# swami1995/diff-qp-mpc

Hardware: AMD Instinct MI355X
Metric: QPs/sec (fwd+bwd), batch=4096 n=3 m=3 T=5 (higher is better)
Workload: dtype f64; 1 GPU; random dense QP family R (SURVEY 8d), configs[0] shape at the BASELINE metric batch: B=4096/GPU nz=30 nineq=30 neq=15; global_batch=4096, n_state=3, n_ctrl=3, T=5, parallelism=batch-shard x1, termination=batch (the reference's batch-coupled rule, parity-safe)

## Files before the change

diff-qp-mpc_amd/_lib.py:

```python
import ctypes
import os

from . import _build

_dp = ctypes.c_void_p


class dqp_dims(ctypes.Structure):
    _fields_ = [("nbatch", ctypes.c_int32), ("nz", ctypes.c_int32), ("nineq", ctypes.c_int32),
                ("neq", ctypes.c_int32),
                ("stride_Q", ctypes.c_int64), ("stride_p", ctypes.c_int64),
                ("stride_G", ctypes.c_int64), ("stride_h", ctypes.c_int64),
                ("stride_A", ctypes.c_int64), ("stride_b", ctypes.c_int64)]


class dqp_opts(ctypes.Structure):
    _fields_ = [("eps", ctypes.c_double), ("stall_tol", ctypes.c_double),
                ("max_iter", ctypes.c_int32),
                ("not_improved_lim", ctypes.c_int32), ("flags", ctypes.c_uint32),
                ("reserved", ctypes.c_int32),
                ("dyn_id", ctypes.c_int32), ("dyn_T", ctypes.c_int32), ("dyn_dt", ctypes.c_double),
                ("dyn_x0", ctypes.c_void_p)]


DQP_OK = 0
DQP_FLAG_DENSE_BACKWARD = 1
DQP_FLAG_GENERIC_ONLY = 2
DQP_FLAG_NO_NULLSPACE = 4
DQP_FLAG_RIC_GLOBAL_WS = 64
DQP_FLAG_BACKWARD_CTX = 8
DQP_FLAG_BATCH_TERMINATION = 16
DQP_FLAG_HISTORY_ONLY = 32
DQP_FLAG_STRICT_GET_STEP = 128
DQP_FLAG_STAGEWISE = 256
DQP_STATUS_Q_NOT_PD = 1
DQP_STATUS_A_RANK_DEF = 2
DQP_MAX_DIM = 64
DQP_MAX_DIM_LARGE = 512
SHARED_GRAD_KC = 64

SYMBOLS = ("dqp_version", "dqp_error_string", "dqp_workspace_bytes", "dqp_termination_bytes",
           "dqp_qp_forward", "dqp_qp_backward", "dqp_qp_backward_shared_bytes", "dqp_qp_backward_shared", "dqp_term_local_masks", "dqp_qp_forward_finish", "dqp_mpc_assemble", "dqp_mpc_assemble_backward",
           "dqp_mpc_qp_supported", "dqp_mpc_qp_workspace_bytes", "dqp_mpc_qp_host_n_state", "dqp_mpc_qp_termination_bytes", "dqp_mpc_qp_forward", "dqp_mpc_qp_backward", "dqp_mpc_line_search", "dqp_mpc_rollout_backward",
           "dqp_al_newton_step", "dqp_al_chol_solve", "dqp_al_assemble", "dqp_al_merit",
           "dqp_al_newton_solve_bytes", "dqp_al_newton_solve",
           "dqp_al_outer_update", "dqp_al_banded_factor_bytes", "dqp_al_banded_newton_step", "dqp_al_banded_solve",
           "dqp_al_banded_newton_step_jac", "dqp_al_banded_jac_factor_bytes", "dqp_al_lane_group", "dqp_al_mpc_solve_bytes", "dqp_al_mpc_solve",
           "dqp_al_mpc_solve_fused_supported", "dqp_al_mpc_solve_fused_bytes", "dqp_al_mpc_solve_fused",
           "dqp_mpc_qp_stepped_workspace_bytes", "dqp_mpc_qp_stepped_termination_bytes", "dqp_mpc_qp_forward_stepped", "dqp_trace_begin", "dqp_trace_end",
           "dqp_dyn_sizes", "dqp_dyn_step", "dqp_dyn_jacobian", "dqp_dyn_forward_dynamics",
           "dqp_dyn_forward_derivatives")
DQP_DYN = {"pendulum1l": 1, "cartpole1l": 2, "cartpole2l": 3, "pendulum_euler": 4, "pendulum_dx": 5,
           "rexquadrotor": 6, "integrator": 7}


class dqp_al_mpc_dims(ctypes.Structure):
    _fields_ = [("nbatch", ctypes.c_int32), ("n_state", ctypes.c_int32), ("n_ctrl", ctypes.c_int32),
                ("T", ctypes.c_int32)]


class dqp_al_dims(ctypes.Structure):
    _fields_ = [("nbatch", ctypes.c_int32), ("nz", ctypes.c_int32), ("ncon", ctypes.c_int32),
                ("reserved", ctypes.c_int32)]


class dqp_mpc_dims(ctypes.Structure):
    _fields_ = [("nbatch", ctypes.c_int32), ("n_state", ctypes.c_int32), ("n_ctrl", ctypes.c_int32),
                ("T", ctypes.c_int32), ("has_bounds", ctypes.c_int32), ("dyn_id", ctypes.c_int32),
                ("n_state_host", ctypes.c_int32)]



class dqp_trace_record(ctypes.Structure):
    _fields_ = [("kernel", ctypes.c_char * 248), ("ms", ctypes.c_float), ("reserved", ctypes.c_int32)]


_lib = None


def path():
    return os.environ.get("DQP_HIP_LIBRARY") or _build.SO


def load():
    global _lib
    if _lib is not None:
        return _lib
    so = path()
    if not os.path.exists(so):
        raise RuntimeError(
            "diff_qp_mpc_amd: %s is missing. Build it with `python -c 'import __graft_entry__ as g; "
            "g.build()'` (hipcc --offload-arch=gfx950). There is no CPU fallback." % so)
    try:
        lib = ctypes.CDLL(so)
    except OSError as e:
        raise RuntimeError("diff_qp_mpc_amd: cannot load %s: %s" % (so, e))
    lib.dqp_version.restype = ctypes.c_int
    lib.dqp_error_string.restype = ctypes.c_char_p
    lib.dqp_error_string.argtypes = [ctypes.c_int]
    lib.dqp_workspace_bytes.restype = ctypes.c_size_t
    lib.dqp_workspace_bytes.argtypes = [ctypes.POINTER(dqp_dims)]
    lib.dqp_qp_forward.restype = ctypes.c_int
    lib.dqp_termination_bytes.restype = ctypes.c_size_t
    lib.dqp_termination_bytes.argtypes = [ctypes.POINTER(dqp_dims), ctypes.POINTER(dqp_opts)]
    lib.dqp_qp_forward.argtypes = [ctypes.POINTER(dqp_dims), ctypes.POINTER(dqp_opts)] + [_dp] * 15
    lib.dqp_term_local_masks.restype = ctypes.c_int
    lib.dqp_term_local_masks.argtypes = [ctypes.POINTER(dqp_dims), ctypes.POINTER(dqp_opts)] + [_dp] * 3
    lib.dqp_qp_forward_finish.restype = ctypes.c_int
    lib.dqp_qp_forward_finish.argtypes = [ctypes.POINTER(dqp_dims), ctypes.POINTER(dqp_opts)] + [_dp] * 16
    lib.dqp_qp_backward.restype = ctypes.c_int
    lib.dqp_qp_backward.argtypes = [ctypes.POINTER(dqp_dims), ctypes.POINTER(dqp_opts)] + [_dp] * 17
    lib.dqp_qp_backward_shared_bytes.restype = ctypes.c_size_t
    lib.dqp_qp_backward_shared_bytes.argtypes = [ctypes.POINTER(dqp_dims)]
    lib.dqp_qp_backward_shared.restype = ctypes.c_int
    lib.dqp_qp_backward_shared.argtypes = [ctypes.POINTER(dqp_dims), ctypes.POINTER(dqp_opts)] + [_dp] * 18
    lib.dqp_mpc_assemble.restype = ctypes.c_int
    lib.dqp_mpc_assemble.argtypes = [ctypes.POINTER(dqp_mpc_dims)] + [_dp] * 14
# ... 115 lines not shown
```

diff-qp-mpc_amd/csrc/dqp_common.h:

```cpp
#ifndef DQP_COMMON_H_
#define DQP_COMMON_H_
#include <hip/hip_runtime.h>
#include <stdint.h>

#include "../../include/dqp.h"
#include "dqp_trace.h"

namespace dqp {

constexpr int WAVE = 64;

struct KParams {
    const double *Q, *p, *G, *h, *A, *b;
    long long sQ, sp, sG, sh, sA, sb;
    double *zhat, *lam, *nu, *slack, *best_resid;
    const double *zin, *lamin, *nuin, *slackin, *gin;
    double *dQ, *dp, *dG, *dh, *dA, *db;
    int32_t *info;
    double *workspace;
    unsigned long long *stamps;
    int B, N, M, E;
    int ldz, ldm, lde, ldt;
    double eps, stallTol;
    int maxIter, notImprovedLim;
    unsigned flags;
    double *hist;
    const int32_t *cap;
    int histIters;
    int dynId, dynT, dynN, dynM;
    double dynDt;
    const double *dynX0;
    const double *mC, *mc, *mF, *mf, *mx0, *mul, *muu;
    double *mdC, *mdc, *mdF, *mdf, *mdx0;
    int mn, mm, mT;
    double *snap;
    const double *histIn;
    const double *extRy;
    int itBegin, itEnd;
};

constexpr int TERM_HDR = 8;

constexpr int TERM_MAXIT = 64;
constexpr int TERM_ACC_BYTES = 3 * 8 + TERM_HDR * 4;

__device__ __forceinline__ void hist_put(const KParams &P, long long qp, int it, double resid, double mu)
{
    double2 *h = reinterpret_cast<double2 *>(P.hist) + (long long)it * P.B + qp;
    *h = make_double2(resid, mu);
}
__device__ __forceinline__ void hist_fill(const KParams &P, long long qp, int iters)
{
    const double nan = __builtin_nan("");
    for (int it = iters; it < P.histIters; ++it)
        reinterpret_cast<double2 *>(P.hist)[(long long)it * P.B + qp] = make_double2(nan, nan);
}
__device__ __forceinline__ void term_zero_acc(const KParams &P)
{
    if (P.hist && blockIdx.x == 0) {
        unsigned *a = reinterpret_cast<unsigned *>(P.hist + (long long)P.B * P.histIters * 2);
        for (int i = threadIdx.x; i < TERM_ACC_BYTES / 4; i += blockDim.x) a[i] = 0u;
    }
}

__device__ __forceinline__ bool term_flagged(const KParams &P, long long qp) { return P.cap[TERM_HDR + qp] >= P.cap[0]; }

size_t term_bytes(int B, int maxIter, int snapDim);
int term_decide(const KParams &P, void *term, void *stream);
int term_local_masks(const KParams &P, void *term, unsigned long long *masks, void *stream);
int term_decide_global(const KParams &P, void *term, const unsigned long long *masks, void *stream);
void term_bind_pass1(KParams &P, void *term, int snapDim);
void term_bind_pass2(KParams &P, void *term);


#ifdef DQP_STAMPS
extern unsigned long long *g_debug_stamps;
#endif
int r16_forward(const KParams &P, void *stream);
int r16_backward(const KParams &P, void *stream);
int r16n_forward(const KParams &P, void *stream);
long long r16n_workspace_doubles(int N, int M, int E);
int r16n_snapshot_doubles(int N, int M, int E);
bool ric_supported(int n_state, int n_ctrl);
long long ric_workspace_doubles(int n_state, int n_ctrl, int T);
int ric_forward(const KParams &P, void *stream);
long long ric_stepped_workspace_doubles(int n_state, int n_ctrl, int T, int B);
int ric_forward_stepped(const KParams &P, void *stream);
int ric_backward(const KParams &P, void *stream);
int ric_snapshot_doubles(int n_state, int n_ctrl, int T);
int ric_finish(const KParams &P, void *stream);
bool ricw_supported(int n_state, int n_ctrl);
long long ricw_workspace_doubles(int n_state, int n_ctrl, int T);
int ricw_forward(const KParams &P, void *stream);
long long ricw_stepped_workspace_doubles(int n_state, int n_ctrl, int T, int B);
int ricw_forward_stepped(const KParams &P, void *stream);
int ricw_backward(const KParams &P, void *stream);
int ricw_snapshot_doubles(int n_state, int n_ctrl, int T);
#define DQP_RIC_HOST16_SIZES X(15, 1) X(14, 2) X(13, 3) X(11, 5) X(10, 6) X(9, 7) X(8, 8)
#define DQP_RIC_HOSTW_SIZES X(31, 1) X(30, 2) X(29, 3) X(28, 4) X(27, 5) X(26, 6) X(25, 7)
#define DQP_RIC_HOST_SIZES DQP_RIC_HOST16_SIZES DQP_RIC_HOSTW_SIZES
#define DQP_RIC_HOST_PART_IDS PART(0) PART(1) PART(2) PART(3) PART(4) PART(5) PART(6) PART(7) PART(8)
enum { RIC_HOST_FORWARD = 0, RIC_HOST_STEPPED = 1, RIC_HOST_BACKWARD = 2 };
#define PART(k) int ric_host_run_##k(int op, const KParams &P, void *stream);
DQP_RIC_HOST_PART_IDS
#undef PART
bool stage_supported(int n_state, int n_ctrl);
bool stage_native(int n_state, int n_ctrl);
int stage_q(int n_state, int n_ctrl);
long long stage_layout_doubles(int n_state, int n_ctrl, int T);
int stage_forward(const KParams &P, void *stream);
int stage_forward_stepped(const KParams &P, void *stream);
int stage_backward(const KParams &P, void *stream);
struct PadRegion {
    double *C, *F, *c, *tau, *g, *dc, *f, *df, *nu, *ry, *x0, *dx0, *dC, *dF;
};
long long pad_kernel_doubles(int n_host, int n_ctrl, int T, int B, bool stepped);
long long pad_region_doubles(int n_host, int n_ctrl, int T, int B);
PadRegion pad_region(double *base, int n_host, int n_ctrl, int T, int B);
int pad_pack(int n, int n_host, int m, int T, int B, const PadRegion &R, const double *C, const double *c, const double *F,
             const double *f, const double *x0, const double *tau, const double *nu, const double *g, const double *ry,
             void *stream);
int pad_unpack(int n, int n_host, int m, int T, int B, const PadRegion &R, double *tau, double *nu, double *dC, double *dc,
               double *dF, double *df, double *dx0, void *stream);
long long big_workspace_doubles(int N, int M, int E);
bool big_fits(int N, int M, int E);
int big_forward(const KParams &P, void *stream);
int big_backward(const KParams &P, void *stream);

int al_banded_newton_step_keep(const dqp_al_mpc_dims *d, int dyn_id, double dt, const double *xu, const double *x0,
                               const double *Qdiag, const double *q, const double *lam, const double *rho,
                               const double *u_lower, const double *u_upper, double *update, void *factor, int32_t *info,
                               void *stream, int keep);
int r16n_backward(const KParams &P, void *stream);

}
#endif
```

diff-qp-mpc_amd/csrc/dqp_pdipm.hip:

```cpp

#include <hip/hip_runtime.h>
#include <math.h>
#include <stdint.h>

#include "dqp_common.h"
#include "dqp_dyn_models.h"

using namespace dqp;

namespace {

#define WSYNC() __syncthreads()

__device__ __forceinline__ double bcast(double v, int src)
{
    int lo = __double2loint(v), hi = __double2hiint(v);
    lo = __builtin_amdgcn_readlane(lo, src);
    hi = __builtin_amdgcn_readlane(hi, src);
    return __hiloint2double(hi, lo);
}

template <int CTRL> __device__ __forceinline__ double dppd(double v)
{
    return __builtin_amdgcn_update_dpp(v, v, CTRL, 0xf, 0xf, true);
// ... 641 lines not shown
template <typename K>
int launch(K kernel, const KParams &P, size_t lds_bytes, void *stream)
{
    if (P.B == 0) return DQP_OK;
    if (lds_bytes > 64 * 1024) {
        if (hipFuncSetAttribute(reinterpret_cast<const void *>(kernel),
                                hipFuncAttributeMaxDynamicSharedMemorySize,
                                (int)lds_bytes) != hipSuccess)
            return DQP_ERR_LAUNCH;
    }
    DQP_LAUNCH(kernel, dim3(P.B), dim3(WAVE), lds_bytes, (hipStream_t)stream, P);
    return hipGetLastError() == hipSuccess ? DQP_OK : DQP_ERR_LAUNCH;
}

}

#ifdef DQP_STAMPS
namespace dqp { unsigned long long *g_debug_stamps = nullptr; }
#endif

extern "C" {

#ifdef DQP_STAMPS
__attribute__((visibility("default"))) void dqp_debug_set_stamps(void *dev_ptr)
{
    dqp::g_debug_stamps = (unsigned long long *)dev_ptr;
}
#endif

__attribute__((visibility("default"))) int dqp_version(void) { return DQP_VERSION; }

__attribute__((visibility("default"))) const char *dqp_error_string(int code)
{
    switch (code) {
    case DQP_OK: return "ok";
    case DQP_ERR_BAD_ARG: return "bad argument";
    case DQP_ERR_TOO_LARGE: return "problem too large for the fused one-wavefront kernels";
    case DQP_ERR_LAUNCH: return "HIP kernel launch failed";
    case DQP_ERR_NO_DEVICE: return "no HIP device";
    default: return "unknown error";
    }
}

__attribute__((visibility("default"))) size_t dqp_workspace_bytes(const dqp_dims *d)
{
    if (!d || d->nbatch <= 0) return 0;
    if (d->nz > DQP_MAX_DIM || d->nineq > DQP_MAX_DIM || d->neq > DQP_MAX_DIM) {
        if (d->nz > DQP_MAX_DIM_LARGE || d->nineq > DQP_MAX_DIM_LARGE || d->neq > DQP_MAX_DIM_LARGE) return 0;
        return (size_t)d->nbatch * (size_t)dqp::big_workspace_doubles(d->nz, d->nineq, d->neq) * sizeof(double);
    }
    return (size_t)d->nbatch * (size_t)dqp::r16n_workspace_doubles(d->nz, d->nineq, d->neq) * sizeof(double);
}

__attribute__((visibility("default"))) size_t
dqp_termination_bytes(const dqp_dims *d, const dqp_opts *o)
{
    if (!d || d->nbatch <= 0 || !o || !(o->flags & DQP_FLAG_BATCH_TERMINATION)) return 0;
    return dqp::term_bytes(d->nbatch, o->max_iter, dqp::r16n_snapshot_doubles(d->nz, d->nineq, d->neq));
}

static int forward_once(const KParams &P, size_t lds, void *workspace, void *stream);

__attribute__((visibility("default"))) int
dqp_qp_forward(const dqp_dims *dims, const dqp_opts *opts, const double *Q, const double *p,
               const double *G, const double *h, const double *A, const double *b, double *zhat,
               double *lam, double *nu, double *slack, int32_t *info, double *best_resid,
               void *workspace, void *termination, void *stream)
{
    KParams P = {};
    size_t lds = 0;
    int rc = fill_params(dims, opts, P, lds);
    if (rc != DQP_OK) return rc;
    if (P.B == 0) return DQP_OK;
    if (!Q || !p || !G || !h || !zhat || !lam || !slack) return DQP_ERR_BAD_ARG;
    P.workspace = (double *)workspace;
    if (P.E > 0 && (!A || !b || !nu)) return DQP_ERR_BAD_ARG;
    P.Q = Q; P.p = p; P.G = G; P.h = h; P.A = A; P.b = b;
    P.zhat = zhat; P.lam = lam; P.nu = nu; P.slack = slack;
    P.info = info; P.best_resid = best_resid;
    if (!(P.flags & DQP_FLAG_BATCH_TERMINATION)) return forward_once(P, lds, workspace, stream);
    if (!termination || P.maxIter < 1 || P.maxIter > 64) return DQP_ERR_BAD_ARG;
    P.eps = opts ? opts->eps : 1e-12;
    const bool nullspace = workspace && !(P.flags & (DQP_FLAG_GENERIC_ONLY | DQP_FLAG_NO_NULLSPACE)) && !P.dynId && !is_big(P);
    term_bind_pass1(P, termination, nullspace ? r16n_snapshot_doubles(P.N, P.M, P.E) : 0);
    if ((rc = forward_once(P, lds, workspace, stream)) != DQP_OK) return rc;
    if (P.flags & DQP_FLAG_HISTORY_ONLY) return DQP_OK;
    if ((rc = term_decide(P, termination, stream)) != DQP_OK) return rc;
    term_bind_pass2(P, termination);
    return forward_once(P, lds, workspace, stream);
}

__attribute__((visibility("default"))) int
dqp_term_local_masks(const dqp_dims *dims, const dqp_opts *opts, void *termination, uint64_t *masks, void *stream)
{
    KParams P = {};
    size_t lds = 0;
    int rc = fill_params(dims, opts, P, lds);
    if (rc != DQP_OK) return rc;
    if (!(P.flags & DQP_FLAG_BATCH_TERMINATION) || !termination || !masks || P.maxIter < 1 || P.maxIter > 64)
        return DQP_ERR_BAD_ARG;
    if (P.B == 0) return hipMemsetAsync(masks, 0, 24, (hipStream_t)stream) == hipSuccess ? DQP_OK : DQP_ERR_LAUNCH;
    P.eps = opts ? opts->eps : 1e-12;
    return term_local_masks(P, termination, (unsigned long long *)masks, stream);
}

__attribute__((visibility("default"))) int
dqp_qp_forward_finish(const dqp_dims *dims, const dqp_opts *opts, const double *Q, const double *p,
                      const double *G, const double *h, const double *A, const double *b, double *zhat,
                      double *lam, double *nu, double *slack, int32_t *info, double *best_resid,
                      void *workspace, void *termination, const uint64_t *masks, void *stream)
{
    KParams P = {};
    size_t lds = 0;
    int rc = fill_params(dims, opts, P, lds);
    if (rc != DQP_OK) return rc;
    if (P.B == 0) return DQP_OK;
    if (!(P.flags & DQP_FLAG_BATCH_TERMINATION) || !termination || !masks || P.maxIter < 1 || P.maxIter > 64)
        return DQP_ERR_BAD_ARG;
    if (!Q || !p || !G || !h || !zhat || !lam || !slack) return DQP_ERR_BAD_ARG;
    if (P.E > 0 && (!A || !b || !nu)) return DQP_ERR_BAD_ARG;
    P.workspace = (double *)workspace;
    P.Q = Q; P.p = p; P.G = G; P.h = h; P.A = A; P.b = b;
    P.zhat = zhat; P.lam = lam; P.nu = nu; P.slack = slack;
    P.info = info; P.best_resid = best_resid;
    P.eps = opts ? opts->eps : 1e-12;
    const bool nullspace = workspace && !(P.flags & (DQP_FLAG_GENERIC_ONLY | DQP_FLAG_NO_NULLSPACE)) && !P.dynId && !is_big(P);
    term_bind_pass1(P, termination, nullspace ? r16n_snapshot_doubles(P.N, P.M, P.E) : 0);
    if ((rc = term_decide_global(P, termination, (const unsigned long long *)masks, stream)) != DQP_OK) return rc;
    term_bind_pass2(P, termination);
    return forward_once(P, lds, workspace, stream);
}

static int forward_once(const KParams &P, size_t lds, void *workspace, void *stream)
{
    int rc;
    if (is_big(P)) return workspace ? big_forward(P, stream) : DQP_ERR_BAD_ARG;
    if (!(P.flags & DQP_FLAG_GENERIC_ONLY) && !P.dynId) {
        rc = (workspace && !(P.flags & DQP_FLAG_NO_NULLSPACE)) ? r16n_forward(P, stream) : 1;
        if (rc == 1) rc = r16_forward(P, stream);
        if (rc != 1) return rc;
    }
    const int mx = P.N > P.M ? (P.N > P.E ? P.N : P.E) : (P.M > P.E ? P.M : P.E);
    if (mx <= 16) return launch(qp_forward_kernel<16>, P, lds, stream);
    if (mx <= 32) return launch(qp_forward_kernel<32>, P, lds, stream);
    return launch(qp_forward_kernel<64>, P, lds, stream);
}

enum { MPC_NONE = 0, MPC_R16N = 1, MPC_RIC = 2, MPC_RICW = 3, MPC_PAD = 4 };

static long long stage_ws_doubles(int n, int m, int T)
{
    return ric_supported(n, m) ? ric_workspace_doubles(n, m, T) : ricw_workspace_doubles(n, m, T);
}

static int mpc_params(const dqp_mpc_dims *md, const dqp_opts *opts, KParams &P, size_t &lds, int &kind)
{
    kind = MPC_NONE;
    if (!md || md->T < 2 || md->n_state < 1 || md->n_ctrl < 1 || !md->has_bounds || md->nbatch < 0) return DQP_ERR_BAD_ARG;
    dqp_dims d = {};
    d.nbatch = md->nbatch;
    d.nz = md->T * (md->n_state + md->n_ctrl);
    d.nineq = 2 * md->T * md->n_ctrl;
    d.neq = md->T * md->n_state;
    if (md->n_state_host) {
        const int np = md->n_state_host, m = md->n_ctrl;
        if (md->dyn_id || np < md->n_state || !stage_supported(np, m)) return DQP_ERR_BAD_ARG;
        if (md->T > 200000 || stage_layout_doubles(np, m, md->T) * 8 * 4 > 0x7fffffffLL) return DQP_ERR_TOO_LARGE;
        P.stamps = nullptr;
        P.B = d.nbatch; P.N = md->T * (np + m); P.M = d.nineq; P.E = md->T * np;
        fill_opts(opts, P);
// ... 286 lines not shown
```

diff-qp-mpc_amd/csrc/dqp_r16n.hip:

```cpp

#include "dqp_r16_prims.h"

namespace dqp {
namespace r16n {

using namespace dqp::r16;

template <int N_, int M_, int E_> struct Cfg {
    static constexpr int N = N_, M = M_, E = E_, R = N_ - E_;
    static constexpr int SN = slots(N_), SM = slots(M_), SR = slots(N_ - E_);
    static constexpr int SE = E_ > 0 ? slots(E_) : 1, EC = E_ > 0 ? E_ : 1;
    static constexpr bool PARK = slots(N_) >= 3;
#ifndef DQP_R16N_PARK_WU
#define DQP_R16N_PARK_WU 1
#endif
    static constexpr bool PARKWU = PARK || DQP_R16N_PARK_WU;
#ifndef DQP_R16N_PIN_ALL
#define DQP_R16N_PIN_ALL 1
#endif
    static constexpr bool PIN = PARK || DQP_R16N_PIN_ALL;
#ifndef DQP_R16N_SPLIT_ALL
#define DQP_R16N_SPLIT_ALL 0
#endif
    static constexpr bool SPLIT = PARK || DQP_R16N_SPLIT_ALL;
// ... 829 lines not shown
        if (r == 0) {
            if (P.info) { P.info[2 * qp] = st.status; P.info[2 * qp + 1] = iters; }
            if (P.best_resid) P.best_resid[qp] = best;
        }
    }
}

template <class C>
__global__ __launch_bounds__(64) void forward_kernel(KParams P)
{
    constexpr int N = C::N, M = C::M, E = C::E, R = C::R;
    constexpr int SN = C::SN, SM = C::SM, SE = C::SE, SR = C::SR;
    extern __shared__ __attribute__((aligned(16))) double sm[];
    const int lane = threadIdx.x, r = lane & 15, qrow = lane >> 4;
    long long qp = (long long)blockIdx.x * 4 + qrow;
    bool live = qp < P.B;
    if (!live) qp = P.B - 1;
    int maxIter = P.maxIter;
    const bool batch = (P.flags & DQP_FLAG_BATCH_TERMINATION) != 0;
    const bool strict = (P.flags & DQP_FLAG_STRICT_GET_STEP) != 0;
    if (P.cap) {
        maxIter = min(maxIter, P.cap[0]);
        live = live && term_flagged(P, qp);
        if (__builtin_amdgcn_ballot_w64(live) == 0) return;
    }
    double *lds = sm + qrow * C::ldsQPpad;
    double *dummy = lds + C::oDummy + r;

    term_zero_acc(P);
    State<C> st;
    STAMP(P, 0);
    setup<C>(P, qp, r, lds, st);
    STAMP(P, 15);

    bool inM[SM], inR[SR];
#pragma unroll
    for (int s = 0; s < SM; ++s) inM[s] = r + 16 * s < M;
#pragma unroll
    for (int s = 0; s < SR; ++s) inR[s] = r + 16 * s < R;

    double T[SM][M], rdu[SM];
    double w[SR], s_[SM], z[SM];
    double cc = 1.0, delta = 0.0;
    {
        double one[SM], hp[SM], cp[SR], g[SM], gtz[SR];
#pragma unroll
        for (int s = 0; s < SM; ++s) one[s] = inM[s] ? 1.0 : 0.0;
        vec_get<SM>(lds + C::oHp, hp, M, r);
        vec_get<SR>(lds + C::oCp, cp, R, r);
        mul_Gz<C>(st, cp, g);
#pragma unroll
        for (int s = 0; s < SM; ++s) g[s] = inM[s] ? -hp[s] - g[s] : 0.0;
        __builtin_amdgcn_sched_barrier(0);
        factor_T<C>(lds, T, st.rdiag, one, rdu, r);
        lu_solve<SM, M>(T, rdu, g, r);
        __builtin_amdgcn_sched_barrier(0);
        mul_GzT<C>(st, g, gtz, r);
#pragma unroll
        for (int s = 0; s < SR; ++s) w[s] = inR[s] ? -cp[s] - gtz[s] : 0.0;
        double ms = INFINITY, mz = INFINITY;
#pragma unroll
        for (int s = 0; s < SM; ++s) {
            z[s] = inM[s] ? g[s] : 0.0;
            s_[s] = -z[s];
            ms = fmin(ms, inM[s] ? s_[s] : INFINITY);
            mz = fmin(mz, inM[s] ? z[s] : INFINITY);
        }
        ms = row_min(ms); mz = row_min(mz);
#pragma unroll
        for (int s = 0; s < SM; ++s) {
            if (ms < 0.0 && inM[s]) s_[s] -= ms - 1.0;
            if (mz < 0.0 && inM[s]) z[s] -= mz - 1.0;
        }
        delta = mz < 0.0 ? 1.0 - mz : 0.0;
        if (r == 0) P.workspace[qp * (long long)C::wsQP + C::wDl] = delta;
    }

    double gz[SR];
    mul_GzT<C>(st, z, gz, r);
    STAMP(P, 6);
    double best = INFINITY, bestc = 1.0;
    bool have_best = false, done = false;
    int nNot = 0, iters = 0;

    for (int it = 0; it < maxIter; ++it) {
        double rw[SR], rz[SM];
        {
            double cp[SR], hp[SM], gw[SM];
            vec_get<SR>(lds + C::oCp, cp, R, r);
            vec_get<SM>(lds + C::oHp, hp, M, r);
            mul_Gz<C>(st, w, gw);
#pragma unroll
            for (int s = 0; s < SR; ++s) rw[s] = inR[s] ? w[s] + cp[s] + gz[s] : 0.0;
#pragma unroll
            for (int s = 0; s < SM; ++s) rz[s] = inM[s] ? gw[s] + s_[s] - hp[s] : 0.0;
        }
        double sz = 0.0, nz2 = 0.0;
#pragma unroll
        for (int s = 0; s < SM; ++s) { sz = fma(s_[s], z[s], sz); nz2 = fma(rz[s], rz[s], nz2); }
        double nx2 = rx_norm2_partial<C>(st, lds, rw, cc * delta, r);
        sz = row_sum(sz); nz2 = row_sum(nz2); nx2 = row_sum(nx2);
        const double mu = fabs(sz * (1.0 / M));
        const double resid = sqrt(nz2) + sqrt(nx2) + M * mu;
        if (!done) {
            iters = it + 1;
            if (!have_best || resid < best) {
                nNot = 0; have_best = true; best = resid; bestc = cc;
                vec_put<SR>(lds + C::oBw, w, R, r, dummy);
                vec_put<SM>(lds + C::oBs, s_, M, r, dummy);
                vec_put<SM>(lds + C::oBz, z, M, r, dummy);
                if (P.snap && live) {
                    double *sp = P.snap + ((long long)it * P.B + qp) * C::snapDim;
#pragma unroll
                    for (int s = 0; s < SR; ++s)
                        if (inR[s]) sp[r + 16 * s] = w[s];
#pragma unroll
                    for (int s = 0; s < SM; ++s)
                        if (inM[s]) { sp[R + r + 16 * s] = s_[s]; sp[R + M + r + 16 * s] = z[s]; }
                    if (r == 0) sp[R + 2 * M] = cc;
                }
            } else {
                nNot += 1;
            }
            if (batch) {
                if (P.hist && r == 0 && live) hist_put(P, qp, it, resid, mu);
                done = !(fabs(resid) < INFINITY);
            } else if ((nNot >= P.notImprovedLim && best < P.stallTol) || best < P.eps || mu > 1e32 ||
                       !(fabs(resid) < INFINITY))
                done = true;
        }
        if (__builtin_amdgcn_ballot_w64(!done) == 0) break;
        if (it == 1) STAMP(P, 9);

        double dza[SM], dsa[SM];
        {
            double gu[SM];
            mul_Gz<C>(st, rw, gu);
#pragma unroll
            for (int s = 0; s < SM; ++s) dza[s] = rz[s] - s_[s] - gu[s];
        }
        __builtin_amdgcn_sched_barrier(0);
        double dinv[SM];
#pragma unroll
        for (int s = 0; s < SM; ++s) dinv[s] = inM[s] ? s_[s] * frcp(z[s]) : 0.0;
        factor_T<C>(lds, T, st.rdiag, dinv, rdu, r);
        if (it == 1) STAMP(P, 10);
        lu_solve<SM, M>(T, rdu, dza, r);
        if (it == 1) STAMP(P, 11);
        double rzv[SM], rsv[SM];
#pragma unroll
        for (int s = 0; s < SM; ++s) {
            rzv[s] = inM[s] ? frcp(z[s]) : 0.0;
            rsv[s] = inM[s] ? frcp(s_[s]) : 0.0;
        }
        double tm = 0.0;
#pragma unroll
        for (int s = 0; s < SM; ++s) {
            dsa[s] = (-z[s] - dza[s]) * dinv[s];
            tm = fmax(tm, fmax(-dza[s] * rzv[s], -dsa[s] * rsv[s]));
        }
        bool zero_step = false;
        if (strict) {
#pragma unroll
            for (int s = 0; s < SM; ++s) zero_step |= inM[s] && (dza[s] == 0.0 || dsa[s] == 0.0);
        }
        double alpha = frcp(fmax(row_max(tm), 1.0));
        double t3 = 0.0;
#pragma unroll
        for (int s = 0; s < SM; ++s)
            t3 = fma(fma(alpha, dsa[s], s_[s]), fma(alpha, dza[s], z[s]), t3);
        t3 = row_sum(t3);
        double sig = t3 / sz;
        sig = sig * sig * sig;
        double rsc[SM], dzc[SM], dz[SM], ds[SM];
#pragma unroll
        for (int s = 0; s < SM; ++s) {
            rsc[s] = fma(dsa[s], dza[s], -mu * sig) * rsv[s];
            dzc[s] = -rsc[s] * dinv[s];
        }
        lu_solve<SM, M>(T, rdu, dzc, r);
        if (it == 1) STAMP(P, 12);
        tm = 0.0;
#pragma unroll
        for (int s = 0; s < SM; ++s) {
            dz[s] = dza[s] + dzc[s];
            ds[s] = fma(-rsc[s] - dzc[s], dinv[s], dsa[s]);
            tm = fmax(tm, fmax(-dz[s] * rzv[s], -ds[s] * rsv[s]));
        }
        if (strict) {
#pragma unroll
            for (int s = 0; s < SM; ++s) zero_step |= inM[s] && (dz[s] == 0.0 || ds[s] == 0.0);
            if ((__builtin_amdgcn_ballot_w64(zero_step) >> (lane & 48)) & 0xffffull) done = true;
        }
        __builtin_amdgcn_sched_barrier(0);
        double gtd[SR];
        mul_GzT<C>(st, dz, gtd, r);
        alpha = frcp(fmax(row_max(tm) * (1.0 / 0.999), 1.0));
        if (!done) {
#pragma unroll
            for (int s = 0; s < SR; ++s) {
                w[s] = fma(alpha, -rw[s] - gtd[s], w[s]);
                gz[s] = fma(alpha, gtd[s], gz[s]);
            }
#pragma unroll
            for (int s = 0; s < SM; ++s) { s_[s] = fma(alpha, ds[s], s_[s]); z[s] = fma(alpha, dz[s], z[s]); }
            cc *= (1.0 - alpha);
        }
        if (it == 1) STAMP(P, 13);
        if (it == 0) STAMP(P, 8);
    }
    STAMP(P, 7);

    if (P.hist && r == 0 && live) hist_fill(P, qp, iters);
    epilogue<C>(P, qp, r, lds, st, bestc, delta, iters, best, live, true);
    STAMP(P, 14);
}

template <class C>
__device__ __forceinline__ void load_ctx(const KParams &P, long long qp, int r, double *lds, State<C> &st)
{
    constexpr int N = C::N, M = C::M, E = C::E, R = C::R;
    constexpr int SN = C::SN, SM = C::SM, SE = C::SE;
    st.status = DQP_STATUS_OK;
    {
        const double *ws = P.workspace + qp * (long long)C::wsQP;
        for (int e = r; e < C::tailsz; e += 16) lds[C::oTl + e] = ws[C::wTl + e];
        for (int e = r; e < tri(N); e += 16) lds[C::oLq + e] = ws[C::wLq + e];
#pragma unroll
        for (int s = 0; s < SM; ++s) {
            const int i = r + 16 * s, ic = i < M ? i : M - 1;
#pragma unroll
            for (int c = 0; c < N; ++c) {
                const double v = ws[C::wG + c * M + ic];
                st.Gh[s][c] = (16 * s + 15 >= M) ? mask_hi(v, i < M) : v;
            }
        }
#pragma unroll
        for (int s = 0; s < SE; ++s) {
            const int k = r + 16 * s, kc = k < E ? k : E - 1;
#pragma unroll
            for (int c = 0; c < N; ++c) st.Ah[s][c] = 0.0;
#pragma unroll
            for (int e = 0; e < E; ++e) {
                const double v = ws[C::wU + e * E + kc];
                st.Ah[s][R + e] = k < E ? v : 0.0;
            }
            const double t = ws[C::wTau + kc], u = ws[C::wRdu + kc];
            st.tau[s] = k < E ? t : 0.0;
            st.rdu1[s] = k < E ? u : 0.0;
        }
#pragma unroll
        for (int s = 0; s < SN; ++s) {
            const int i = r + 16 * s;
            const double v = ws[C::wRdq + (i < N ? i : N - 1)];
            st.rdq[s] = i < N ? v : 0.0;
        }
    }
}

template <class C>
__global__ __launch_bounds__(64) void finish_kernel(KParams P)
{
    constexpr int M = C::M, E = C::E, R = C::R;
    constexpr int SM = C::SM, SE = C::SE, SR = C::SR;
    extern __shared__ __attribute__((aligned(16))) double sm[];
    const int lane = threadIdx.x, r = lane & 15, qrow = lane >> 4;
    long long qp = (long long)blockIdx.x * 4 + qrow;
    bool live = qp < P.B;
    if (!live) qp = P.B - 1;
    live = live && term_flagged(P, qp);
    if (__builtin_amdgcn_ballot_w64(live) == 0) return;
    const int cap = min(P.maxIter, P.cap[0]);
    double *lds = sm + qrow * C::ldsQPpad;
    double *dummy = lds + C::oDummy + r;
    State<C> st;
    load_ctx<C>(P, qp, r, lds, st);
    const double *ws = P.workspace + qp * (long long)C::wsQP;
#pragma unroll
    for (int s = 0; s < SE; ++s) {
        const int k = r + 16 * s, kc = k < E ? k : (E > 0 ? E - 1 : 0);
        const double a = ws[C::wXy + kc], b = ws[C::wPy + kc], c = ws[C::wW1 + kc];
        st.xy[s] = (E > 0 && k < E) ? a : 0.0;
        st.py[s] = (E > 0 && k < E) ? b : 0.0;
        st.w1[s] = (E > 0 && k < E) ? c : 0.0;
    }
    const double delta = ws[C::wDl];
    const double2 *h = reinterpret_cast<const double2 *>(P.histIn) + qp;
    double best = h[0].x;
    int arg = 0;
    for (int it = 1; it < cap; ++it) {
        const double v = h[(long long)it * P.B].x;
        if (v < best) { best = v; arg = it; }
    }
    const double *sp = P.snap + ((long long)arg * P.B + qp) * C::snapDim;
    double bw[SR], bs[SM], bz[SM];
#pragma unroll
    for (int s = 0; s < SR; ++s) { const int i = r + 16 * s; const double v = sp[i < R ? i : 0]; bw[s] = i < R ? v : 0.0; }
#pragma unroll
    for (int s = 0; s < SM; ++s) {
        const int i = r + 16 * s, ic = i < M ? i : 0;
        const double a = sp[R + ic], b = sp[R + M + ic];
        bs[s] = i < M ? a : 0.0;
        bz[s] = i < M ? b : 0.0;
    }
    const double bestc = sp[R + 2 * M];
    vec_put<SR>(lds + C::oBw, bw, R, r, dummy);
    vec_put<SM>(lds + C::oBs, bs, M, r, dummy);
    vec_put<SM>(lds + C::oBz, bz, M, r, dummy);
    st.status = P.info ? P.info[2 * qp] : DQP_STATUS_OK;
    epilogue<C>(P, qp, r, lds, st, bestc, delta, cap, best, live, false);
}

template <class C>
__global__ __launch_bounds__(64) void backward_kernel(KParams P)
{
    constexpr int N = C::N, M = C::M, E = C::E, R = C::R;
    constexpr int SN = C::SN, SM = C::SM, SE = C::SE, SR = C::SR;
    extern __shared__ __attribute__((aligned(16))) double sm[];
    const int lane = threadIdx.x, r = lane & 15, qrow = lane >> 4;
    long long qp = (long long)blockIdx.x * 4 + qrow;
    const bool live = qp < P.B;
    if (!live) qp = P.B - 1;
    double *lds = sm + qrow * C::ldsQPpad;

    State<C> st;
    load_ctx<C>(P, qp, r, lds, st);
    __syncthreads();

    bool inN[SN], inM[SM], inE[SE];
#pragma unroll
    for (int s = 0; s < SN; ++s) inN[s] = r + 16 * s < N;
#pragma unroll
    for (int s = 0; s < SM; ++s) inM[s] = r + 16 * s < M;
#pragma unroll
    for (int s = 0; s < SE; ++s) inE[s] = r + 16 * s < E;

    double zh[SN], g[SN], lam[SM], dinv[SM], nu[SE];
#pragma unroll
    for (int s = 0; s < SN; ++s) {
        zh[s] = inN[s] ? P.zin[qp * N + r + 16 * s] : 0.0;
        g[s] = inN[s] ? P.gin[qp * N + r + 16 * s] : 0.0;
    }
#pragma unroll
    for (int s = 0; s < SM; ++s) {
        lam[s] = inM[s] ? P.lamin[qp * M + r + 16 * s] : 0.0;
        const double sl = inM[s] ? P.slackin[qp * M + r + 16 * s] : 1.0;
        if (P.flags & DQP_FLAG_DENSE_BACKWARD) dinv[s] = inM[s] ? sl / lam[s] : 0.0;
        else dinv[s] = inM[s] ? fmax(sl, 1e-8) / fmax(lam[s], 1e-8) : 0.0;
    }
#pragma unroll
    for (int s = 0; s < SE; ++s) nu[s] = (E > 0 && inE[s]) ? P.nuin[qp * E + r + 16 * s] : 0.0;

    tri_solve<SN, N>(lds + C::oLq, st.rdq, g, r);
    double gy[SE];
#pragma unroll
// ... 183 lines not shown
```

diff-qp-mpc_amd/csrc/dqp_term.hip:

```cpp
#include "dqp_common.h"

namespace dqp {

namespace {

constexpr int MAXIT = TERM_MAXIT;
struct Acc {
    unsigned long long improved;
    unsigned long long notbelow;
    unsigned long long notabove;
};
static_assert(sizeof(Acc) + TERM_HDR * sizeof(int32_t) == TERM_ACC_BYTES, "layout shared with dqp_common.h");

inline size_t hist_bytes(int B, int maxIter) { return (size_t)B * maxIter * 2 * sizeof(double); }

__device__ __forceinline__ unsigned long long wave_or_u64(unsigned long long v)
{
#pragma unroll
    for (int off = 32; off > 0; off >>= 1) v |= __shfl_xor(v, off, 64);
    return v;
}

__device__ __forceinline__ int rule_stop(unsigned long long ai, unsigned long long anb, unsigned long long ana, int maxIter,
                                         int notImprovedLim)
{
    int nNot = 0;
    for (int it = 0; it < maxIter; ++it) {
        if (it == 0 || ((ai >> it) & 1ull)) nNot = 0;
        else nNot += 1;
        if (nNot == notImprovedLim || !((anb >> it) & 1ull) || !((ana >> it) & 1ull)) return it + 1;
    }
    return maxIter;
}

constexpr int SCAN_CHUNK = 32;
__global__ __launch_bounds__(64) void term_scan_kernel(const double2 *hist, Acc *acc, int32_t *hdr,
                                                       int B, int maxIter, int notImprovedLim, double eps,
                                                       int decide)
{
    const int lane = threadIdx.x;
    const long long qp = (long long)blockIdx.x * blockDim.x + lane;
    const bool live = qp < B;
    unsigned long long imp = 0ull, nb = 0ull, na = 0ull;
    if (live) {
        const double2 *h = hist + qp;
        double best = 0.0;
        int arg = 0;
        for (int it0 = 0; it0 < maxIter; it0 += SCAN_CHUNK) {
            double2 v[SCAN_CHUNK];
#pragma unroll
            for (int k = 0; k < SCAN_CHUNK; ++k) v[k] = h[(long long)min(it0 + k, maxIter - 1) * B];
#pragma unroll
            for (int k = 0; k < SCAN_CHUNK; ++k) {
                const int it = it0 + k;
                if (it < maxIter) {
                    if (it == 0) best = v[k].x;
                    else if (v[k].x < best) { best = v[k].x; arg = it; imp |= 1ull << it; }
                    if (!(best < eps)) nb |= 1ull << it;
                    if (!(v[k].y > 1e32)) na |= 1ull << it;
                }
            }
        }
        hdr[TERM_HDR + qp] = arg;
    }
    imp = wave_or_u64(imp); nb = wave_or_u64(nb); na = wave_or_u64(na);
    if (lane < 3) {
        const unsigned long long m = lane == 0 ? imp : (lane == 1 ? nb : na);
        unsigned long long *dst = lane == 0 ? &acc->improved : (lane == 1 ? &acc->notbelow : &acc->notabove);
        if (m) atomicOr(dst, m);
    }
    if (!decide) return;
    __threadfence();
    int last = 0;
    if (lane == 0) last = (atomicAdd(&hdr[2], 1) == (int)gridDim.x - 1);
    last = __shfl(last, 0, 64);
    if (!last) return;
    __threadfence();
    if (lane == 0) {
        const unsigned long long ai = __hip_atomic_load(&acc->improved, __ATOMIC_RELAXED, __HIP_MEMORY_SCOPE_AGENT);
        const unsigned long long anb = __hip_atomic_load(&acc->notbelow, __ATOMIC_RELAXED, __HIP_MEMORY_SCOPE_AGENT);
        const unsigned long long ana = __hip_atomic_load(&acc->notabove, __ATOMIC_RELAXED, __HIP_MEMORY_SCOPE_AGENT);
        hdr[0] = rule_stop(ai, anb, ana, maxIter, notImprovedLim);
    }
}

__global__ __launch_bounds__(64) void term_decide_kernel(const unsigned long long *masks, int32_t *hdr, int maxIter,
                                                         int notImprovedLim)
{
    if (threadIdx.x == 0) hdr[0] = rule_stop(masks[0], masks[1], masks[2], maxIter, notImprovedLim);
}

inline Acc *acc_of(void *term, int B, int maxIter) { return (Acc *)((char *)term + hist_bytes(B, maxIter)); }
inline int32_t *hdr_of(void *term, int B, int maxIter) { return (int32_t *)((char *)acc_of(term, B, maxIter) + sizeof(Acc)); }

inline size_t snap_offset(int B, int maxIter)
{
    const size_t o = hist_bytes(B, maxIter) + sizeof(Acc) + (size_t)(TERM_HDR + B) * sizeof(int32_t);
    return (o + 15) & ~(size_t)15;
}

}

size_t term_bytes(int B, int maxIter, int snapDim)
{
    if (B <= 0 || maxIter <= 0) return 0;
    return snap_offset(B, maxIter) + (size_t)B * maxIter * (snapDim > 0 ? snapDim : 0) * sizeof(double);
}

void term_bind_pass1(KParams &P, void *term, int snapDim)
{
    P.hist = (double *)term;
    P.histIters = P.maxIter;
    P.cap = nullptr;
    P.histIn = nullptr;
    P.snap = snapDim > 0 ? (double *)((char *)term + snap_offset(P.B, P.maxIter)) : nullptr;
}

void term_bind_pass2(KParams &P, void *term)
{
    P.hist = nullptr;
    P.histIn = (const double *)term;
    P.cap = hdr_of(term, P.B, P.maxIter);
}

int term_decide(const KParams &P, void *term, void *stream)
{
    const int blocks = (P.B + 63) / 64;
    DQP_LAUNCH(term_scan_kernel, dim3(blocks), dim3(64), 0, (hipStream_t)stream,
                       (const double2 *)term, acc_of(term, P.B, P.maxIter), hdr_of(term, P.B, P.maxIter),
                       P.B, P.maxIter, P.notImprovedLim, P.eps, 1);
    return hipGetLastError() == hipSuccess ? DQP_OK : DQP_ERR_LAUNCH;
}

int term_local_masks(const KParams &P, void *term, unsigned long long *masks, void *stream)
{
    const int blocks = (P.B + 63) / 64;
    DQP_LAUNCH(term_scan_kernel, dim3(blocks), dim3(64), 0, (hipStream_t)stream,
                       (const double2 *)term, acc_of(term, P.B, P.maxIter), hdr_of(term, P.B, P.maxIter),
                       P.B, P.maxIter, P.notImprovedLim, P.eps, 0);
    if (hipMemcpyAsync(masks, acc_of(term, P.B, P.maxIter), 3 * sizeof(unsigned long long), hipMemcpyDeviceToDevice,
                       (hipStream_t)stream) != hipSuccess)
        return DQP_ERR_LAUNCH;
    return hipGetLastError() == hipSuccess ? DQP_OK : DQP_ERR_LAUNCH;
}

int term_decide_global(const KParams &P, void *term, const unsigned long long *masks, void *stream)
{
    DQP_LAUNCH(term_decide_kernel, dim3(1), dim3(64), 0, (hipStream_t)stream, masks,
                       hdr_of(term, P.B, P.maxIter), P.maxIter, P.notImprovedLim);
    return hipGetLastError() == hipSuccess ? DQP_OK : DQP_ERR_LAUNCH;
}

}
```

include/dqp.h:

```cpp
#ifndef DQP_H_
#define DQP_H_

#include <stddef.h>
#include <stdint.h>

#ifdef __cplusplus
extern "C" {
#endif

#define DQP_VERSION 303
#define DQP_MAX_DIM 64
#define DQP_MAX_DIM_LARGE 512

enum {
    DQP_OK = 0,
    DQP_ERR_BAD_ARG = -1,
    DQP_ERR_TOO_LARGE = -2,
    DQP_ERR_LAUNCH = -3,
    DQP_ERR_NO_DEVICE = -4
};

enum {
    DQP_STATUS_OK = 0,
    DQP_STATUS_Q_NOT_PD = 1,
    DQP_STATUS_A_RANK_DEF = 2
};

#define DQP_FLAG_DENSE_BACKWARD 1u

#define DQP_FLAG_GENERIC_ONLY 2u
#define DQP_FLAG_BACKWARD_CTX 8u
#define DQP_FLAG_BATCH_TERMINATION 16u
#define DQP_FLAG_HISTORY_ONLY 32u
#define DQP_FLAG_NO_NULLSPACE 4u
#define DQP_FLAG_RIC_GLOBAL_WS 64u

#define DQP_FLAG_STRICT_GET_STEP 128u

#define DQP_FLAG_STAGEWISE 256u

typedef struct dqp_dims {
    int32_t nbatch;
    int32_t nz;
    int32_t nineq;
    int32_t neq;
    int64_t stride_Q, stride_p, stride_G, stride_h, stride_A, stride_b;
} dqp_dims;

typedef struct dqp_opts {
    double eps;
    double stall_tol;
    int32_t max_iter;
    int32_t not_improved_lim;
    uint32_t flags;
    int32_t reserved;
    int32_t dyn_id;
    int32_t dyn_T;
    double dyn_dt;
    const double *dyn_x0;
} dqp_opts;

int dqp_version(void);
const char *dqp_error_string(int code);

size_t dqp_workspace_bytes(const dqp_dims *dims);

size_t dqp_termination_bytes(const dqp_dims *dims, const dqp_opts *opts);

int dqp_term_local_masks(const dqp_dims *dims, const dqp_opts *opts, void *termination, uint64_t *masks,
                         void *stream);
int dqp_qp_forward_finish(const dqp_dims *dims, const dqp_opts *opts, const double *Q, const double *p,
                          const double *G, const double *h, const double *A, const double *b, double *zhat,
                          double *lam, double *nu, double *slack, int32_t *info, double *best_resid,
                          void *workspace, void *termination, const uint64_t *masks, void *stream);

int dqp_qp_forward(const dqp_dims *dims, const dqp_opts *opts,
                   const double *Q, const double *p, const double *G, const double *h,
                   const double *A, const double *b,
                   double *zhat, double *lam, double *nu, double *slack,
                   int32_t *info, double *best_resid,
                   void *workspace, void *termination, void *stream);

int dqp_qp_backward(const dqp_dims *dims, const dqp_opts *opts,
                    const double *Q, const double *G, const double *A,
                    const double *zhat, const double *lam, const double *nu,
                    const double *slack, const double *dl_dzhat,
                    double *dQ, double *dp, double *dG, double *dh, double *dA, double *db,
                    int32_t *info, void *workspace, void *stream);

size_t dqp_qp_backward_shared_bytes(const dqp_dims *dims);
int dqp_qp_backward_shared(const dqp_dims *dims, const dqp_opts *opts,
                           const double *Q, const double *G, const double *A,
                           const double *zhat, const double *lam, const double *nu,
                           const double *slack, const double *dl_dzhat,
                           double *dQ, double *dp, double *dG, double *dh, double *dA, double *db,
                           int32_t *info, void *workspace, void *reduce_ws, void *stream);


typedef struct dqp_mpc_dims {
    int32_t nbatch;
    int32_t n_state;
    int32_t n_ctrl;
    int32_t T;
    int32_t has_bounds;
    int32_t dyn_id;
    int32_t n_state_host;
} dqp_mpc_dims;

int dqp_mpc_assemble(const dqp_mpc_dims *dims, const double *C, const double *c, const double *F,
                     const double *f, const double *x0, const double *u_lower,
                     const double *u_upper, double *Q, double *p, double *G, double *h,
                     double *A, double *b, void *stream);

int dqp_mpc_assemble_backward(const dqp_mpc_dims *dims, const double *dQ, const double *dp,
                              const double *dA, const double *db, double *dC, double *dc,
                              double *dF, double *df, double *dx0, void *stream);

int dqp_mpc_qp_supported(const dqp_mpc_dims *dims);
size_t dqp_mpc_qp_workspace_bytes(const dqp_mpc_dims *dims);
int32_t dqp_mpc_qp_host_n_state(const dqp_mpc_dims *dims);
size_t dqp_mpc_qp_termination_bytes(const dqp_mpc_dims *dims, const dqp_opts *opts);
int dqp_mpc_qp_forward(const dqp_mpc_dims *dims, const dqp_opts *opts, const double *C, const double *c,
// ... 141 lines not shown
```

Baseline: 16.14 million QPs/sec.

## Fuse batch termination decision into pass-two kernel via per-block slot masks

Adds an opt-in path where the first forward pass writes per-block OR-reduced improvement/below-eps/not-diverged bitmasks into slots, and every block of the second pass reduces all slots itself to compute the batch stop iteration. This removes the separate term_scan kernel launch between the two passes. In exchange every block redundantly scans all slots, and the path only runs when the new DQP_FLAG_TERM_SLOTS flag is set.

```diff
diff --git a/diff-qp-mpc_amd/_lib.py b/diff-qp-mpc_amd/_lib.py
--- a/diff-qp-mpc_amd/_lib.py
+++ b/diff-qp-mpc_amd/_lib.py
@@ -33,6 +33,7 @@
 DQP_FLAG_HISTORY_ONLY = 32
 DQP_FLAG_STRICT_GET_STEP = 128
 DQP_FLAG_STAGEWISE = 256
+DQP_FLAG_TERM_SLOTS = 512
 DQP_STATUS_Q_NOT_PD = 1
 DQP_STATUS_A_RANK_DEF = 2
 DQP_MAX_DIM = 64
diff --git a/diff-qp-mpc_amd/csrc/dqp_common.h b/diff-qp-mpc_amd/csrc/dqp_common.h
--- a/diff-qp-mpc_amd/csrc/dqp_common.h
+++ b/diff-qp-mpc_amd/csrc/dqp_common.h
@@ -27,6 +27,7 @@
     double *hist;
     const int32_t *cap;
     int histIters;
+    int termFused;
     int dynId, dynT, dynN, dynM;
     double dynDt;
     const double *dynX0;
@@ -43,6 +44,35 @@
 
 constexpr int TERM_MAXIT = 64;
 constexpr int TERM_ACC_BYTES = 3 * 8 + TERM_HDR * 4;
+constexpr int TERM_FUSED_MAXIT = 32;
+constexpr int TERM_FUSED_MAXB = 8192;
+
+__host__ __device__ inline size_t term_hist_bytes(int B, int iters) { return (size_t)B * iters * 2 * sizeof(double); }
+__host__ __device__ inline size_t term_slot_offset(int B, int iters)
+{
+    return (term_hist_bytes(B, iters) + TERM_ACC_BYTES + (size_t)B * sizeof(int32_t) + 15) & ~(size_t)15;
+}
+__host__ __device__ inline int term_slot_count(int B) { return (B + 3) / 4; }
+__host__ __device__ inline int32_t *term_hdr(const double *base, int B, int iters)
+{
+    return (int32_t *)((char *)base + term_hist_bytes(B, iters) + 3 * 8);
+}
+__host__ __device__ inline uint4 *term_slots(const double *base, int B, int iters)
+{
+    return (uint4 *)((char *)base + term_slot_offset(B, iters));
+}
+
+__host__ __device__ inline int term_rule_stop(unsigned long long ai, unsigned long long anb, unsigned long long ana,
+                                              int maxIter, int notImprovedLim)
+{
+    int nNot = 0;
+    for (int it = 0; it < maxIter; ++it) {
+        if (it == 0 || ((ai >> it) & 1ull)) nNot = 0;
+        else nNot += 1;
+        if (nNot == notImprovedLim || !((anb >> it) & 1ull) || !((ana >> it) & 1ull)) return it + 1;
+    }
+    return maxIter;
+}
 
 __device__ __forceinline__ void hist_put(const KParams &P, long long qp, int it, double resid, double mu)
 {
@@ -57,10 +87,55 @@
 }
 __device__ __forceinline__ void term_zero_acc(const KParams &P)
 {
-    if (P.hist && blockIdx.x == 0) {
+    if (P.hist && !P.termFused && blockIdx.x == 0) {
         unsigned *a = reinterpret_cast<unsigned *>(P.hist + (long long)P.B * P.histIters * 2);
         for (int i = threadIdx.x; i < TERM_ACC_BYTES / 4; i += blockDim.x) a[i] = 0u;
     }
+}
+
+__device__ __forceinline__ void term_slot_put(const KParams &P, long long qp, bool live, int iters, double best, unsigned imp,
+                                              unsigned nb, unsigned na)
+{
+    const int lane = threadIdx.x & 63;
+    const unsigned ran = iters >= 32 ? ~0u : (1u << iters) - 1u;
+    const unsigned all = P.histIters >= 32 ? ~0u : (1u << P.histIters) - 1u;
+    const unsigned tail = all & ~ran;
+    imp &= ~1u;
+    if (!(best < P.eps)) nb |= tail;
+    na |= tail;
+    if (live && (lane & 15) == 0) term_hdr(P.hist, P.B, P.histIters)[TERM_HDR + qp] = imp ? 31 - __clz(imp) : 0;
+    if (!live) imp = nb = na = 0u;
+    uint4 v;
+    v.x = __builtin_amdgcn_readlane(imp, 0) | __builtin_amdgcn_readlane(imp, 16) | __builtin_amdgcn_readlane(imp, 32) |
+          __builtin_amdgcn_readlane(imp, 48);
+    v.y = __builtin_amdgcn_readlane(nb, 0) | __builtin_amdgcn_readlane(nb, 16) | __builtin_amdgcn_readlane(nb, 32) |
+          __builtin_amdgcn_readlane(nb, 48);
+    v.z = __builtin_amdgcn_readlane(na, 0) | __builtin_amdgcn_readlane(na, 16) | __builtin_amdgcn_readlane(na, 32) |
+          __builtin_amdgcn_readlane(na, 48);
+    v.w = 0u;
+    if (lane == 0) term_slots(P.hist, P.B, P.histIters)[blockIdx.x] = v;
+}
+
+constexpr int TERM_SLOT_CHUNK = 16;
+__device__ __forceinline__ int term_slot_decide(const KParams &P)
+{
+    const int lane = threadIdx.x & 63;
+    const uint4 *slots = term_slots(P.histIn, P.B, P.histIters);
+    const int ns = term_slot_count(P.B);
+    unsigned a = 0u, b = 0u, c = 0u;
+    for (int i0 = 0; i0 < ns; i0 += 64 * TERM_SLOT_CHUNK) {
+        uint4 v[TERM_SLOT_CHUNK];
+#pragma unroll
+        for (int k = 0; k < TERM_SLOT_CHUNK; ++k) v[k] = slots[min(i0 + 64 * k + lane, ns - 1)];
+#pragma unroll
+        for (int k = 0; k < TERM_SLOT_CHUNK; ++k) { a |= v[k].x; b |= v[k].y; c |= v[k].z; }
+    }
+#pragma unroll
+    for (int off = 32; off > 0; off >>= 1) {
+        a |= __shfl_xor(a, off, 64); b |= __shfl_xor(b, off, 64); c |= __shfl_xor(c, off, 64);
+    }
+    a = __builtin_amdgcn_readfirstlane(a); b = __builtin_amdgcn_readfirstlane(b); c = __builtin_amdgcn_readfirstlane(c);
+    return term_rule_stop(a, b, c, P.maxIter, P.notImprovedLim);
 }
 
 __device__ __forceinline__ bool term_flagged(const KParams &P, long long qp) { return P.cap[TERM_HDR + qp] >= P.cap[0]; }
@@ -69,7 +144,7 @@
 int term_decide(const KParams &P, void *term, void *stream);
 int term_local_masks(const KParams &P, void *term, unsigned long long *masks, void *stream);
 int term_decide_global(const KParams &P, void *term, const unsigned long long *masks, void *stream);
-void term_bind_pass1(KParams &P, void *term, int snapDim);
+void term_bind_pass1(KParams &P, void *term, int snapDim, bool fused = false);
 void term_bind_pass2(KParams &P, void *term);
 
 
diff --git a/diff-qp-mpc_amd/csrc/dqp_pdipm.hip b/diff-qp-mpc_amd/csrc/dqp_pdipm.hip
--- a/diff-qp-mpc_amd/csrc/dqp_pdipm.hip
+++ b/diff-qp-mpc_amd/csrc/dqp_pdipm.hip
@@ -747,10 +747,13 @@
     if (!termination || P.maxIter < 1 || P.maxIter > 64) return DQP_ERR_BAD_ARG;
     P.eps = opts ? opts->eps : 1e-12;
     const bool nullspace = workspace && !(P.flags & (DQP_FLAG_GENERIC_ONLY | DQP_FLAG_NO_NULLSPACE)) && !P.dynId && !is_big(P);
-    term_bind_pass1(P, termination, nullspace ? r16n_snapshot_doubles(P.N, P.M, P.E) : 0);
+    const int snapDim = nullspace ? r16n_snapshot_doubles(P.N, P.M, P.E) : 0;
+    const bool fused = snapDim > 0 && (P.flags & DQP_FLAG_TERM_SLOTS) && !(P.flags & DQP_FLAG_HISTORY_ONLY) &&
+                       P.maxIter <= TERM_FUSED_MAXIT && P.B <= TERM_FUSED_MAXB;
+    term_bind_pass1(P, termination, snapDim, fused);
     if ((rc = forward_once(P, lds, workspace, stream)) != DQP_OK) return rc;
     if (P.flags & DQP_FLAG_HISTORY_ONLY) return DQP_OK;
-    if ((rc = term_decide(P, termination, stream)) != DQP_OK) return rc;
+    if (!fused && (rc = term_decide(P, termination, stream)) != DQP_OK) return rc;
     term_bind_pass2(P, termination);
     return forward_once(P, lds, workspace, stream);
 }
diff --git a/diff-qp-mpc_amd/csrc/dqp_r16n.hip b/diff-qp-mpc_amd/csrc/dqp_r16n.hip
--- a/diff-qp-mpc_amd/csrc/dqp_r16n.hip
+++ b/diff-qp-mpc_amd/csrc/dqp_r16n.hip
@@ -935,6 +935,7 @@
     double best = INFINITY, bestc = 1.0;
     bool have_best = false, done = false;
     int nNot = 0, iters = 0;
+    unsigned m_imp = 0u, m_nb = 0u, m_na = 0u;
 
     for (int it = 0; it < maxIter; ++it) {
         double rw[SR], rz[SM];
@@ -959,6 +960,7 @@
             iters = it + 1;
             if (!have_best || resid < best) {
                 nNot = 0; have_best = true; best = resid; bestc = cc;
+                m_imp |= 1u << (it & 31);
                 vec_put<SR>(lds + C::oBw, w, R, r, dummy);
                 vec_put<SM>(lds + C::oBs, s_, M, r, dummy);
                 vec_put<SM>(lds + C::oBz, z, M, r, dummy);
@@ -977,6 +979,8 @@
             }
             if (batch) {
                 if (P.hist && r == 0 && live) hist_put(P, qp, it, resid, mu);
+                if (!(best < P.eps)) m_nb |= 1u << (it & 31);
+                if (!(mu > 1e32)) m_na |= 1u << (it & 31);
                 done = !(fabs(resid) < INFINITY);
             } else if ((nNot >= P.notImprovedLim && best < P.stallTol) || best < P.eps || mu > 1e32 ||
                        !(fabs(resid) < INFINITY))
@@ -1065,6 +1069,7 @@
     STAMP(P, 7);
 
     if (P.hist && r == 0 && live) hist_fill(P, qp, iters);
+    if (P.termFused) term_slot_put(P, qp, live, iters, best, m_imp, m_nb, m_na);
     epilogue<C>(P, qp, r, lds, st, bestc, delta, iters, best, live, true);
     STAMP(P, 14);
 }
@@ -1121,9 +1126,18 @@
     long long qp = (long long)blockIdx.x * 4 + qrow;
     bool live = qp < P.B;
     if (!live) qp = P.B - 1;
-    live = live && term_flagged(P, qp);
+    int istar;
+    if (P.termFused) {
+        const int mine = P.cap[TERM_HDR + qp];
+        istar = term_slot_decide(P);
+        if (blockIdx.x == 0 && lane == 0) const_cast<int32_t *>(P.cap)[0] = istar;
+        live = live && mine >= istar;
+    } else {
+        istar = P.cap[0];
+        live = live && term_flagged(P, qp);
+    }
     if (__builtin_amdgcn_ballot_w64(live) == 0) return;
-    const int cap = min(P.maxIter, P.cap[0]);
+    const int cap = min(P.maxIter, istar);
     double *lds = sm + qrow * C::ldsQPpad;
     double *dummy = lds + C::oDummy + r;
     State<C> st;
diff --git a/diff-qp-mpc_amd/csrc/dqp_term.hip b/diff-qp-mpc_amd/csrc/dqp_term.hip
--- a/diff-qp-mpc_amd/csrc/dqp_term.hip
+++ b/diff-qp-mpc_amd/csrc/dqp_term.hip
@@ -12,25 +12,13 @@
 };
 static_assert(sizeof(Acc) + TERM_HDR * sizeof(int32_t) == TERM_ACC_BYTES, "layout shared with dqp_common.h");
 
-inline size_t hist_bytes(int B, int maxIter) { return (size_t)B * maxIter * 2 * sizeof(double); }
+inline size_t hist_bytes(int B, int maxIter) { return term_hist_bytes(B, maxIter); }
 
 __device__ __forceinline__ unsigned long long wave_or_u64(unsigned long long v)
 {
 #pragma unroll
     for (int off = 32; off > 0; off >>= 1) v |= __shfl_xor(v, off, 64);
     return v;
-}
-
-__device__ __forceinline__ int rule_stop(unsigned long long ai, unsigned long long anb, unsigned long long ana, int maxIter,
-                                         int notImprovedLim)
-{
-    int nNot = 0;
-    for (int it = 0; it < maxIter; ++it) {
-        if (it == 0 || ((ai >> it) & 1ull)) nNot = 0;
-        else nNot += 1;
-        if (nNot == notImprovedLim || !((anb >> it) & 1ull) || !((ana >> it) & 1ull)) return it + 1;
-    }
-    return maxIter;
 }
 
 constexpr int SCAN_CHUNK = 32;
@@ -80,14 +68,14 @@
         const unsigned long long ai = __hip_atomic_load(&acc->improved, __ATOMIC_RELAXED, __HIP_MEMORY_SCOPE_AGENT);
         const unsigned long long anb = __hip_atomic_load(&acc->notbelow, __ATOMIC_RELAXED, __HIP_MEMORY_SCOPE_AGENT);
         const unsigned long long ana = __hip_atomic_load(&acc->notabove, __ATOMIC_RELAXED, __HIP_MEMORY_SCOPE_AGENT);
-        hdr[0] = rule_stop(ai, anb, ana, maxIter, notImprovedLim);
+        hdr[0] = term_rule_stop(ai, anb, ana, maxIter, notImprovedLim);
     }
 }
 
 __global__ __launch_bounds__(64) void term_decide_kernel(const unsigned long long *masks, int32_t *hdr, int maxIter,
                                                          int notImprovedLim)
 {
-    if (threadIdx.x == 0) hdr[0] = rule_stop(masks[0], masks[1], masks[2], maxIter, notImprovedLim);
+    if (threadIdx.x == 0) hdr[0] = term_rule_stop(masks[0], masks[1], masks[2], maxIter, notImprovedLim);
 }
 
 inline Acc *acc_of(void *term, int B, int maxIter) { return (Acc *)((char *)term + hist_bytes(B, maxIter)); }
@@ -95,8 +83,7 @@
 
 inline size_t snap_offset(int B, int maxIter)
 {
-    const size_t o = hist_bytes(B, maxIter) + sizeof(Acc) + (size_t)(TERM_HDR + B) * sizeof(int32_t);
-    return (o + 15) & ~(size_t)15;
+    return term_slot_offset(B, maxIter) + (size_t)term_slot_count(B) * sizeof(uint4);
 }
 
 }
@@ -107,8 +94,9 @@
     return snap_offset(B, maxIter) + (size_t)B * maxIter * (snapDim > 0 ? snapDim : 0) * sizeof(double);
 }
 
-void term_bind_pass1(KParams &P, void *term, int snapDim)
+void term_bind_pass1(KParams &P, void *term, int snapDim, bool fused)
 {
+    P.termFused = fused ? 1 : 0;
     P.hist = (double *)term;
     P.histIters = P.maxIter;
     P.cap = nullptr;
diff --git a/include/dqp.h b/include/dqp.h
--- a/include/dqp.h
+++ b/include/dqp.h
@@ -38,6 +38,8 @@
 #define DQP_FLAG_STRICT_GET_STEP 128u
 
 #define DQP_FLAG_STAGEWISE 256u
+
+#define DQP_FLAG_TERM_SLOTS 512u
 
 typedef struct dqp_dims {
     int32_t nbatch;
```

Result: slower. 15.52 million QPs/sec (-3.9%).
